# nucypher/nufhe

Measured on NVIDIA B200. Metric: bootstrapped gates/sec (NAND) at batch 4096 per GPU, higher is better.
Workload: dtype u64

## Files before the change

### nufhe_b200/csrc/br_fft.cuh

```cuda
#pragma once
#include "br_phases.cuh"
#include <math.h>
#include <string.h>

namespace nb {

constexpr int FFT_M = 512;
constexpr int FFT_STRIDE = FFT_M + FFT_M / 8;
constexpr int FFT_KEY_SPECTRA = 16;
constexpr int FFT_ROW_U64 = FFT_KEY_SPECTRA * FFT_M * 2;
constexpr double FFT_ROUND_MAGIC = 6755399441055744.0;
constexpr double FFT_DIGIT_BIAS = 4503599627370496.0 + 512.0;
constexpr double FFT_SQRT1_2 = 0.70710678118654752440;
NB_HDC double fft_cos16(int j)
{
    return j == 0 ? 1.0 : j == 1 ? 0.9807852804032304491262 : j == 2 ? 0.9238795325112867561282
         : j == 3 ? 0.8314696123025452370788 : j == 4 ? 0.7071067811865475244008 : j == 5 ? 0.5555702330196022247428
         : j == 6 ? 0.3826834323650897717285 : j == 7 ? 0.1950903220161282678483 : 0.0;
}

NB_HD int fft_pos(int i) { return i + (i >> 3); }

struct cplx { double re, im; };

// ... 72 lines not shown
#endif
}
NB_HD cplx ld_c_global(const cplx *p)
{
#if defined(__CUDA_ARCH__)
    const double2 t = __ldg(reinterpret_cast<const double2 *>(p));
    return {t.x, t.y};
#else
    return *p;
#endif
}

template <bool INV> NB_HD cplx c_rot8(cplx a)
{
    return INV ? cplx{d_mul(d_add(a.re, a.im), FFT_SQRT1_2), d_mul(d_sub(a.im, a.re), FFT_SQRT1_2)}
               : cplx{d_mul(d_sub(a.re, a.im), FFT_SQRT1_2), d_mul(d_add(a.re, a.im), FFT_SQRT1_2)};
}
template <bool INV> NB_HD cplx c_rot16(cplx a, int j0)
{
    if (j0 == 4) return c_rot8<INV>(a);
    return c_mul(a, cplx{fft_cos16(j0), INV ? -fft_cos16(8 - j0) : fft_cos16(8 - j0)});
}

template <bool INV> NB_HD void dft8(cplx *x)
{
    auto rot4 = [](cplx a) -> cplx { return INV ? cplx{a.im, -a.re} : cplx{-a.im, a.re}; };
    auto rot8 = [](cplx a) -> cplx { return c_rot8<INV>(a); };
    cplx a[4], b[4];
    for (int j = 0; j < 4; j++) { a[j] = c_add(x[j], x[j + 4]); b[j] = c_sub(x[j], x[j + 4]); }
    b[1] = rot8(b[1]); b[2] = rot4(b[2]); b[3] = rot4(rot8(b[3]));
    cplx a0 = c_add(a[0], a[2]), a1 = c_add(a[1], a[3]), a2 = c_sub(a[0], a[2]), a3 = rot4(c_sub(a[1], a[3]));
    cplx b0 = c_add(b[0], b[2]), b1 = c_add(b[1], b[3]), b2 = c_sub(b[0], b[2]), b3 = rot4(c_sub(b[1], b[3]));
    x[0] = c_add(a0, a1); x[4] = c_sub(a0, a1); x[2] = c_add(a2, a3); x[6] = c_sub(a2, a3);
    x[1] = c_add(b0, b1); x[5] = c_sub(b0, b1); x[3] = c_add(b2, b3); x[7] = c_sub(b2, b3);
}

struct FftTables {
    cplx tw[FFT_M];
    cplx tw2[64];
};

NB_HD void fft_load_tw1(int t, const FftTables &T, cplx *tw)
{
    for (int k0 = 0; k0 < 8; k0++) tw[k0] = ld_c(&T.tw[64 * k0 + t]);
}

NB_HD void fft_fwd1_store(int t, cplx *x, cplx *f, const cplx *tw)
{
    for (int j0 = 1; j0 < 8; j0++) x[j0] = c_rot16<false>(x[j0], j0);
    dft8<false>(x);
    for (int k0 = 0; k0 < 8; k0++) st_c(f + fft_pos(64 * k0 + t), c_mul(x[k0], tw[k0]));
}
NB_HD void fft_fwd2(int t, cplx *f, const FftTables &T)
{
    const int base = 64 * (t >> 3) + (t & 7), j2 = t & 7;
    cplx x[8];
    for (int j1 = 0; j1 < 8; j1++) x[j1] = ld_c(f + fft_pos(base + 8 * j1));
    dft8<false>(x);
    st_c(f + fft_pos(base), x[0]);
    for (int k1 = 1; k1 < 8; k1++) st_c(f + fft_pos(base + 8 * k1), c_mul(x[k1], T.tw2[k1 * 8 + j2]));
}
NB_HD void fft_fwd3(int t, cplx *f)
{
    cplx *g = f + fft_pos(8 * t);
    cplx x[8];
    for (int j2 = 0; j2 < 8; j2++) x[j2] = ld_c(g + j2);
    dft8<false>(x);
    for (int k2 = 0; k2 < 8; k2++) st_c(g + k2, x[k2]);
}
NB_HD void fft_inv3(int t, cplx *f, const FftTables &T)
{
    cplx *g = f + fft_pos(8 * t);
    const int k1 = t & 7;
    cplx x[8];
    for (int k2 = 0; k2 < 8; k2++) x[k2] = ld_c(g + k2);
    dft8<true>(x);
    st_c(g, x[0]);
    for (int j2 = 1; j2 < 8; j2++) st_c(g + j2, c_mul(x[j2], c_conj(T.tw2[j2 * 8 + k1])));
}
NB_HD void fft_inv2(int t, cplx *f)
{
    const int base = 64 * (t >> 3) + (t & 7);
    cplx x[8];
    for (int k1 = 0; k1 < 8; k1++) x[k1] = ld_c(f + fft_pos(base + 8 * k1));
    dft8<true>(x);
    for (int j1 = 0; j1 < 8; j1++) st_c(f + fft_pos(base + 8 * j1), x[j1]);
}
NB_HD void fft_inv1_load(int t, const cplx *f, const cplx *tw, cplx *x)
{
    for (int k0 = 0; k0 < 8; k0++) x[k0] = c_mul(ld_c(f + fft_pos(64 * k0 + t)), c_conj(tw[k0]));
    dft8<true>(x);
    for (int j0 = 1; j0 < 8; j0++) x[j0] = c_rot16<true>(x[j0], j0);
}


template <bool ROTATE>
NB_HD void fft_step_fwd1(int t, const i32 *acc, cplx *f2 , const FftTables &T, int a)
{
    const int ar = a & (NTT_N - 1);
    const bool flip = (a >> 10) & 1;
    u32 tv[16];
    for (int h = 0; h < 16; h++) {
        const int idx = 64 * (h & 7) + t + 512 * (h >> 3);
        const i32 c = ROTATE ? rotate_minus_one(acc, idx, ar, flip) : acc[idx];
        tv[h] = (u32)c + (0x80000000u + (1u << 21));
    }
    cplx tw[8];
    fft_load_tw1(t, T, tw);
#if defined(__CUDA_ARCH__)
#pragma unroll 1
#endif
    for (int j = 0; j < 2; j++) {
        const int sh = 22 - 10 * j;
        cplx x[8];
        for (int j0 = 0; j0 < 8; j0++) {
            const double lo = d_sub(d_from_u32_biased((tv[j0] >> sh) & 1023u), FFT_DIGIT_BIAS);
            const double hi = d_sub(d_from_u32_biased((tv[8 + j0] >> sh) & 1023u), FFT_DIGIT_BIAS);
            x[j0] = cplx{lo, hi};
        }
        fft_fwd1_store(t, x, f2 + j * FFT_STRIDE, tw);
    }
}

NB_HD void fft_step_mac(int i, cplx *w, int stride, int ct, const cplx *key)
{
    cplx k[16];
    for (int s = 0; s < 16; s++) k[s] = ld_c_global(key + s * FFT_M + i);
    const int pos = fft_pos(i);
    for (int c = 0; c < ct; c++) {
        cplx *f = w + c * stride + pos;
        cplx d[4];
        for (int q = 0; q < 4; q++) d[q] = ld_c(f + q * FFT_STRIDE);
        for (int o = 0; o < 4; o++) {
            const int mo = o >> 1, limb = o & 1;
            cplx acc = {0.0, 0.0};
            for (int q = 0; q < 4; q++) acc = c_mac(acc, d[q], k[(q * 2 + mo) * 2 + limb]);
            st_c(f + o * FFT_STRIDE, acc);
        }
    }
}

template <bool ACCUMULATE>
NB_HD void fft_step_inv1(int t, i32 *acc, const cplx *f2 , const FftTables &T,
                         double *err_max = nullptr)
{
    u32 r[16];
    for (int h = 0; h < 16; h++) r[h] = 0;
    cplx tw[8];
    fft_load_tw1(t, T, tw);
#if defined(__CUDA_ARCH__)
#pragma unroll 1
#endif
    for (int limb = 0; limb < 2; limb++) {
        cplx x[8];
        fft_inv1_load(t, f2 + limb * FFT_STRIDE, tw, x);
        const int sh = 16 * limb;
        for (int j0 = 0; j0 < 8; j0++) {
            const cplx y = x[j0];
            r[j0] += d_round_lo32(y.re) << sh;
            r[8 + j0] += d_round_lo32(y.im) << sh;
#if !defined(__CUDA_ARCH__)
            if (err_max) {
                const double e0 = fabs(y.re - nearbyint(y.re)), e1 = fabs(y.im - nearbyint(y.im));
                if (e0 > *err_max) *err_max = e0;
                if (e1 > *err_max) *err_max = e1;
            }
#endif
        }
    }
    for (int h = 0; h < 16; h++) {
        const int idx = 64 * (h & 7) + t + 512 * (h >> 3);
        const u32 v = r[h];
        acc[idx] = ACCUMULATE ? (i32)((u32)acc[idx] + v) : (i32)v;
    }
}

NB_HD void fft_key_phase1(int t, const i32 *k, int limb, cplx *f, const FftTables &T)
{
    cplx x[8];
    for (int j0 = 0; j0 < 8; j0++) {
        const int idx = 64 * j0 + t;
        double v[2];
        for (int h = 0; h < 2; h++) {
            const i32 c = k[idx + 512 * h];
            const i32 lo = (i32)(int16_t)(u32)c;
            const i32 hi = (i32)(((long long)c - lo) >> 16);
            v[h] = (double)(limb ? hi : lo);
        }
        x[j0] = cplx{v[0], v[1]};
    }
    cplx tw[8];
    fft_load_tw1(t, T, tw);
    fft_fwd1_store(t, x, f, tw);
}
NB_HD void fft_key_phase3_store(int t, cplx *f, cplx *out)
{
// ... 9 lines not shown
```

### nufhe_b200/csrc/capi.cu

```cuda
#include <cstdio>
#include <cstdlib>
#include <cstring>
#include <string>
#include <type_traits>
#include <nvtx3/nvToolsExt.h>
#include "../../include/nufhe_b200.h"
#include "kernels.cuh"
#include "fft_kernels.cuh"
#include "tables.h"

using namespace nb;

struct nb_ctx {
    int device;
    cudaStream_t stream;
    u64 *d_ph_fwd, *d_ph_inv;
    u64 *d_ones512;
    int sm_count;
    size_t wide_max;
    size_t wide2_max;
    size_t pair_max;
    int pair_async;
    int max_chunks;
    unsigned *d_sched;
    size_t sched_words;
    int32_t *d_state;
    size_t state_words;
    float *d_cv_blocks;
    size_t cv_words;
    int force_chunks;
    int stagger_cycles;
    int use_fft;
    FftTables *d_fft_tab;
    std::string err;
};

static int fail(nb_ctx *ctx, int code, const std::string &msg)
{
    if (ctx) ctx->err = msg;
    return code;
}

static int check(nb_ctx *ctx, cudaError_t e, const char *what)
{
    if (e == cudaSuccess) return NB_OK;
    return fail(ctx, NB_ECUDA, std::string(what) + ": " + cudaGetErrorString(e));
}

#define NB_TRY(expr)                         \
    do {                                     \
        int _rc = (expr);                    \
        if (_rc != NB_OK) return _rc;        \
    } while (0)

static int launch_check(nb_ctx *ctx, const char *what) { return check(ctx, cudaGetLastError(), what); }

// ... 13 lines not shown
};
struct NvtxRange {
    explicit NvtxRange(const char *name) { nvtxRangePushA(name); }
    ~NvtxRange() { nvtxRangePop(); }
};

#define NB_ON_DEVICE(ctx)                   \
    DeviceGuard _guard((ctx)->device);      \
    NB_TRY(check(ctx, _guard.err, "cudaSetDevice"))

extern "C" {

int nb_ctx_create(int device, void *stream, nb_ctx **out)
{
    if (!out) return NB_EINVAL;
    *out = nullptr;
    nb_ctx *ctx = new nb_ctx();
    ctx->device = device;
    ctx->stream = (cudaStream_t)stream;
    ctx->d_ph_fwd = ctx->d_ph_inv = ctx->d_ones512 = nullptr;
    ctx->d_sched = nullptr; ctx->d_state = nullptr; ctx->sched_words = ctx->state_words = 0;
    ctx->d_cv_blocks = nullptr; ctx->cv_words = 0;
    ctx->d_fft_tab = nullptr;
    *out = ctx;
    NB_ON_DEVICE(ctx);
    cudaDeviceProp prop;
    NB_TRY(check(ctx, cudaGetDeviceProperties(&prop, device), "cudaGetDeviceProperties"));
    ctx->sm_count = prop.multiProcessorCount;
    {
        const char *e = getenv("NUFHE_B200_MAX_CHUNKS");
        ctx->max_chunks = e ? atoi(e) : 50;
        if (ctx->max_chunks < 1) ctx->max_chunks = 1;
        e = getenv("NUFHE_B200_FORCE_CHUNKS");
        ctx->force_chunks = e ? atoi(e) : 0;
        e = getenv("NUFHE_B200_STAGGER");
        ctx->stagger_cycles = e ? atoi(e) : 12000;
        e = getenv("NUFHE_B200_FFT");
        ctx->use_fft = e ? atoi(e) : 1;
    }
    if (const char *e = getenv("NUFHE_B200_FORCE_RARE_PATH")) {
        if (atoi(e)) {
            const u32 zero = 0;
            NB_TRY(check(ctx, cudaMemcpyToSymbol(nb_c_canon_trigger, &zero, sizeof(zero)), "cudaMemcpyToSymbol"));
        }
    }
    if (prop.major < 10)
        return fail(ctx, NB_EUNSUPPORTED, "libnufhe_b200 is built for sm_100a only; device is sm_" +
                                              std::to_string(prop.major) + std::to_string(prop.minor));
    PhaseTables pt;
    NB_TRY(check(ctx, cudaMalloc(&ctx->d_ph_fwd, NTT_N * sizeof(u64)), "cudaMalloc"));
    NB_TRY(check(ctx, cudaMalloc(&ctx->d_ph_inv, NTT_N * sizeof(u64)), "cudaMalloc"));
    NB_TRY(check(ctx, cudaMemcpy(ctx->d_ph_fwd, pt.fwd.data(), NTT_N * sizeof(u64), cudaMemcpyHostToDevice), "memcpy"));
    NB_TRY(check(ctx, cudaMemcpy(ctx->d_ph_inv, pt.inv.data(), NTT_N * sizeof(u64), cudaMemcpyHostToDevice), "memcpy"));
    NB_TRY(check(ctx, cudaMalloc(&ctx->d_ones512, NTT_N * sizeof(u64)), "cudaMalloc"));
    NB_TRY(check(ctx, cudaMemcpy(ctx->d_ones512, pt.ones512.data(), NTT_N * sizeof(u64), cudaMemcpyHostToDevice), "memcpy"));
    {
        FftTables ft;
        make_fft_tables(ft);
        NB_TRY(check(ctx, cudaMalloc(&ctx->d_fft_tab, sizeof(FftTables)), "cudaMalloc"));
        NB_TRY(check(ctx, cudaMemcpy(ctx->d_fft_tab, &ft, sizeof(FftTables), cudaMemcpyHostToDevice), "memcpy"));
    }
    NB_TRY(check(ctx, cudaFuncSetAttribute(blind_rotate_fft_kernel<BrFft>, cudaFuncAttributeMaxDynamicSharedMemorySize,
                                           (int)br_fft_smem_bytes<BrFft>()), "cudaFuncSetAttribute(blind_rotate fft)"));
    NB_TRY(check(ctx, cudaFuncSetAttribute(blind_rotate_kernel<BrDefault>, cudaFuncAttributeMaxDynamicSharedMemorySize,
                                           (int)br_smem_bytes<BrDefault>()), "cudaFuncSetAttribute(blind_rotate)"));
    NB_TRY(check(ctx, cudaFuncSetAttribute(blind_rotate_kernel<BrWide>, cudaFuncAttributeMaxDynamicSharedMemorySize,
                                           (int)br_smem_bytes<BrWide>()), "cudaFuncSetAttribute(blind_rotate wide)"));
    NB_TRY(check(ctx, cudaFuncSetAttribute(blind_rotate_kernel<BrWide2>, cudaFuncAttributeMaxDynamicSharedMemorySize,
                                           (int)br_smem_bytes<BrWide2>()), "cudaFuncSetAttribute(blind_rotate wide2)"));
    NB_TRY(check(ctx, cudaFuncSetAttribute(blind_rotate_pair_kernel<true>, cudaFuncAttributeMaxDynamicSharedMemorySize,
                                           (int)BR_PAIR_SMEM_BYTES), "cudaFuncSetAttribute(blind_rotate pair)"));
    NB_TRY(check(ctx, cudaFuncSetAttribute(blind_rotate_pair_kernel<false>, cudaFuncAttributeMaxDynamicSharedMemorySize,
                                           (int)BR_PAIR_SMEM_BYTES), "cudaFuncSetAttribute(blind_rotate pair)"));
    NB_TRY(check(ctx, cudaFuncSetAttribute(keyswitch_kernel, cudaFuncAttributeMaxDynamicSharedMemorySize,
                                           (int)KS_SMEM_BYTES), "cudaFuncSetAttribute(keyswitch)"));
    {
        const char *e = getenv("NUFHE_B200_WIDE_MAX");
        ctx->wide_max = e ? (size_t)atoll(e) : (size_t)ctx->sm_count * BrWide::CTAS_PER_SM * 17 / 10;
        e = getenv("NUFHE_B200_WIDE2_MAX");
        ctx->wide2_max = e ? (size_t)atoll(e) : (size_t)ctx->sm_count * 3 / 2;
        e = getenv("NUFHE_B200_PAIR_ASYNC");
        ctx->pair_async = e ? atoi(e) : 1;
        e = getenv("NUFHE_B200_PAIR_MAX");
// ... 16 lines not shown
        }
        if (getenv("NUFHE_B200_VERBOSE"))
            fprintf(stderr, "nufhe_b200: device %d, %d SMs; fused-kernel shapes by batch: pair <= %zu, wide2 <= %zu, wide <= %zu\n",
                    ctx->device, ctx->sm_count, ctx->pair_max, ctx->wide2_max, ctx->wide_max);
    }
    NB_TRY(check(ctx, cudaFuncSetAttribute(ntt_forward_kernel<true>, cudaFuncAttributeMaxDynamicSharedMemorySize, (int)ntt_smem_bytes(NTT_RAW_I32_BYTES)), "attr"));
    NB_TRY(check(ctx, cudaFuncSetAttribute(ntt_forward_kernel<false>, cudaFuncAttributeMaxDynamicSharedMemorySize, (int)ntt_smem_bytes(NTT_RAW_U64_BYTES)), "attr"));
    NB_TRY(check(ctx, cudaFuncSetAttribute(ntt_inverse_kernel<true>, cudaFuncAttributeMaxDynamicSharedMemorySize, (int)ntt_smem_bytes(NTT_RAW_U64_BYTES)), "attr"));
    NB_TRY(check(ctx, cudaFuncSetAttribute(ntt_inverse_kernel<false>, cudaFuncAttributeMaxDynamicSharedMemorySize, (int)ntt_smem_bytes(NTT_RAW_U64_BYTES)), "attr"));
    return NB_OK;
}

void nb_ctx_destroy(nb_ctx *ctx)
{
    if (!ctx) return;
    DeviceGuard guard(ctx->device);
    if (ctx->d_ph_fwd) cudaFree(ctx->d_ph_fwd);
    if (ctx->d_ph_inv) cudaFree(ctx->d_ph_inv);
    if (ctx->d_ones512) cudaFree(ctx->d_ones512);
    if (ctx->d_sched) cudaFree(ctx->d_sched);
    if (ctx->d_state) cudaFree(ctx->d_state);
    if (ctx->d_cv_blocks) cudaFree(ctx->d_cv_blocks);
    if (ctx->d_fft_tab) cudaFree(ctx->d_fft_tab);
    delete ctx;
}

const char *nb_last_error(const nb_ctx *ctx) { return ctx ? ctx->err.c_str() : "null context"; }

int nb_ctx_set_stream(nb_ctx *ctx, void *stream)
{
    if (!ctx) return NB_EINVAL;
    ctx->stream = (cudaStream_t)stream;
    return NB_OK;
}

int nb_ctx_synchronize(nb_ctx *ctx)
{
    if (!ctx) return NB_EINVAL;
    NB_ON_DEVICE(ctx);
    return check(ctx, cudaStreamSynchronize(ctx->stream), "cudaStreamSynchronize");
}

const char *nb_build_info(void)
{
    static std::string info;
    if (info.empty()) {
// ... 148 lines not shown
template <class Cfg> static int launch_br_cfg(nb_ctx *ctx, BlindRotateArgs &p)
{
    const size_t slots = (size_t)ctx->sm_count * Cfg::CTAS_PER_SM;
    const size_t chains = (p.batch + Cfg::CT - 1) / Cfg::CT;
    int chunks = p.plain ? 1 : pick_chunks(chains, slots, p.n, ctx->max_chunks);
    if (!p.plain && ctx->force_chunks > 0 && chains > slots) chunks = ctx->force_chunks < p.n ? ctx->force_chunks : p.n;
    p.chains = (unsigned)chains;
    p.steps_per_chunk = p.plain ? 1 : (p.n + chunks - 1) / chunks;
    chunks = p.plain ? 1 : (p.n + p.steps_per_chunk - 1) / p.steps_per_chunk;
    p.chunks = (unsigned)chunks;
    p.sched = nullptr; p.state = nullptr;
    p.sm_count = ctx->sm_count; p.stagger_cycles = ctx->stagger_cycles;
    size_t grid = chains;
    if (chains > slots) {
        const size_t entries = chunks > 1 ? chains * (size_t)chunks : 0;
        NB_TRY(reserve_words(ctx, (void **)&ctx->d_sched, &ctx->sched_words, BR_SCHED_HEADER + entries, sizeof(unsigned)));
        if (chunks > 1)
            NB_TRY(reserve_words(ctx, (void **)&ctx->d_state, &ctx->state_words, chains * Cfg::CT * 2 * NTT_N, sizeof(int32_t)));
        NB_TRY(check(ctx, cudaMemsetAsync(ctx->d_sched, 0, (BR_SCHED_HEADER + entries) * sizeof(unsigned), ctx->stream), "cudaMemsetAsync"));
        p.sched = ctx->d_sched; p.state = ctx->d_state;
        grid = slots;
    }
    if constexpr (std::is_same_v<Cfg, BrFft>)
        blind_rotate_fft_kernel<Cfg><<<(int)grid, Cfg::THREADS, br_fft_smem_bytes<Cfg>(), ctx->stream>>>(p, ctx->d_fft_tab);
    else
        blind_rotate_kernel<Cfg><<<(int)grid, Cfg::THREADS, br_smem_bytes<Cfg>(), ctx->stream>>>(p, ctx->d_ph_fwd, ctx->d_ph_inv);
    return NB_OK;
}

static int launch_br(nb_ctx *ctx, BlindRotateArgs &p)
{
    if (!p.plain && p.n > 0 && p.batch <= ctx->pair_max) {
        p.sched = nullptr; p.state = nullptr; p.chains = (unsigned)p.batch; p.chunks = 1; p.steps_per_chunk = p.n;
        p.sm_count = ctx->sm_count; p.stagger_cycles = 0;
        if (ctx->pair_async) blind_rotate_pair_kernel<true><<<(unsigned)(2 * p.batch), PAIR_THREADS, BR_PAIR_SMEM_BYTES, ctx->stream>>>(p, ctx->d_ph_fwd, ctx->d_ph_inv);
        else blind_rotate_pair_kernel<false><<<(unsigned)(2 * p.batch), PAIR_THREADS, BR_PAIR_SMEM_BYTES, ctx->stream>>>(p, ctx->d_ph_fwd, ctx->d_ph_inv);
        return NB_OK;
    }
    if (p.batch <= ctx->wide2_max) return launch_br_cfg<BrWide2>(ctx, p);
    if (p.batch <= ctx->wide_max) return launch_br_cfg<BrWide>(ctx, p);
    if (ctx->use_fft && !p.plain && !p.bara && p.n > 0) return launch_br_cfg<BrFft>(ctx, p);
    return launch_br_cfg<BrDefault>(ctx, p);
}

extern "C" {

int nb_ctx_reserve(nb_ctx *ctx, size_t batch)
// ... 274 lines not shown
```

### nufhe_b200/csrc/fft_kernels.cuh

```cuda
#pragma once
#include "kernels.cuh"
#include "br_fft.cuh"

namespace nb {

template <int CT_> struct BrFftCfg {
    static constexpr int CT = CT_, THREADS = 128 * CT_;
    static constexpr int CTAS_PER_SM = CT_ <= 2 ? 2 : 1;
};
#ifndef NB_FFT_CT
#define NB_FFT_CT 2
#endif
using BrFft = BrFftCfg<NB_FFT_CT>;

template <class Cfg> constexpr size_t br_fft_smem_bytes()
{
    return (size_t)Cfg::CT * 4 * FFT_STRIDE * sizeof(cplx) + sizeof(FftTables) + (size_t)Cfg::CT * 2 * NTT_N * sizeof(i32) + 64;
}

enum { FFT_CLK_FWD1, FFT_CLK_FWD2, FFT_CLK_FWD3, FFT_CLK_MAC, FFT_CLK_INV3, FFT_CLK_INV2, FFT_CLK_INV1, FFT_CLK_SYNC,
       FFT_CLK_OTHER, FFT_CLK_STEPS, FFT_CLK_SLOTS };
#ifdef NB_FFT_PHASE_CLOCKS
constexpr int FFT_CLK_CTAS = 1024;
__device__ unsigned long long g_fft_phase_clocks[FFT_CLK_CTAS][FFT_CLK_SLOTS];
__shared__ unsigned long long s_fft_clk[FFT_CLK_SLOTS];
struct FftClocks {
    long long t = 0;
    NB_D void start() { t = clock64(); }
    NB_D void mark(int k) { const long long n = clock64(); if (threadIdx.x == 0) s_fft_clk[k] += n - t; t = n; }
    NB_D void flush(int tid)
    {
        if (tid == 0 && blockIdx.x < FFT_CLK_CTAS)
            for (int k = 0; k < FFT_CLK_SLOTS; k++) g_fft_phase_clocks[blockIdx.x][k] += s_fft_clk[k];
    }
};
#else
struct FftClocks {
    NB_D void start() {}
    NB_D void mark(int) {}
    NB_D void flush(int) {}
};
#endif

template <class Cfg>
NB_D void br_fft_step(cplx *w, const FftTables &T, i32 *acc, const int *rot, const cplx *__restrict__ key, int tid, FftClocks &clk)
{
    constexpr int TH = Cfg::THREADS;
    {
        const int pm = tid >> 6;
        fft_step_fwd1<true>(tid & 63, acc + pm * NTT_N, w + pm * 2 * FFT_STRIDE, T, rot[pm >> 1]);
    }
    clk.mark(FFT_CLK_FWD1);
    __syncthreads();
    clk.mark(FFT_CLK_SYNC);
#pragma unroll 1
    for (int it = 0; it < 2; it++) { const int task = it * TH + tid; fft_fwd2(task & 63, w + (task >> 6) * FFT_STRIDE, T); }
    clk.mark(FFT_CLK_FWD2);
    __syncthreads();
    clk.mark(FFT_CLK_SYNC);
#pragma unroll 1
    for (int it = 0; it < 2; it++) { const int task = it * TH + tid; fft_fwd3(task & 63, w + (task >> 6) * FFT_STRIDE); }
    clk.mark(FFT_CLK_FWD3);
    __syncthreads();
    clk.mark(FFT_CLK_SYNC);
#pragma unroll 1
    for (int i = tid; i < FFT_M; i += TH) fft_step_mac(i, w, 4 * FFT_STRIDE, Cfg::CT, key);
    clk.mark(FFT_CLK_MAC);
    __syncthreads();
    clk.mark(FFT_CLK_SYNC);
#pragma unroll 1
    for (int it = 0; it < 2; it++) { const int task = it * TH + tid; fft_inv3(task & 63, w + (task >> 6) * FFT_STRIDE, T); }
    clk.mark(FFT_CLK_INV3);
    __syncthreads();
    clk.mark(FFT_CLK_SYNC);
#pragma unroll 1
    for (int it = 0; it < 2; it++) { const int task = it * TH + tid; fft_inv2(task & 63, w + (task >> 6) * FFT_STRIDE); }
    clk.mark(FFT_CLK_INV2);
    __syncthreads();
    clk.mark(FFT_CLK_SYNC);
    {
        const int pp = tid >> 6;
        fft_step_inv1<true>(tid & 63, acc + pp * NTT_N, w + pp * 2 * FFT_STRIDE, T);
    }
    clk.mark(FFT_CLK_INV1);
}

template <class Cfg>
__global__ void __launch_bounds__(Cfg::THREADS, Cfg::CTAS_PER_SM) blind_rotate_fft_kernel(BlindRotateArgs p, const FftTables *__restrict__ tab_g)
{
    extern __shared__ __align__(16) unsigned char smem_raw[];
    cplx *w = reinterpret_cast<cplx *>(smem_raw);
    FftTables &T = *reinterpret_cast<FftTables *>(w + Cfg::CT * 4 * FFT_STRIDE);
    i32 *acc = reinterpret_cast<i32 *>(&T + 1);
    int *rot = reinterpret_cast<int *>(acc + Cfg::CT * 2 * NTT_N);
    __shared__ unsigned s_item, s_entry;
    const int tid = threadIdx.x;
    FftClocks clk;
#ifdef NB_FFT_PHASE_CLOCKS
    if (tid < FFT_CLK_SLOTS) s_fft_clk[tid] = 0;
#endif
    for (int i = tid; i < (int)(sizeof(FftTables) / 16); i += Cfg::THREADS)
        reinterpret_cast<double2 *>(&T)[i] = reinterpret_cast<const double2 *>(tab_g)[i];
    const cplx *key0 = reinterpret_cast<const cplx *>(p.bk + (size_t)p.n * BK_ROW_U64);
    constexpr int KEY_ROW_CPLX = FFT_KEY_SPECTRA * FFT_M;
    const unsigned total = p.chains * p.chunks;
    constexpr int ACC_WORDS = Cfg::CT * 2 * NTT_N;
    if (Cfg::CTAS_PER_SM > 1 && !p.sched && p.stagger_cycles > 0 && blockIdx.x >= (unsigned)p.sm_count) {
        if (tid == 0) {
            const long long t0 = clock64();
            while (clock64() - t0 < p.stagger_cycles) { }
        }
    }
    __syncthreads();

    for (unsigned item = blockIdx.x;; ) {
        if (p.sched) {
            __syncthreads();
            if (tid == 0) s_item = atomicAdd(p.sched, 1u);
            __syncthreads();
            item = s_item;
        }
        if (item >= total) break;
        unsigned chunk = 0, chain = item;
        if (p.sched && item >= p.chains) {
// ... 87 lines not shown
```

### nufhe_b200/csrc/host_emul.cpp

```cpp
#include <cstring>
#include <vector>
#include "tables.h"

using namespace nb;

extern "C" {

void emul_ntt_forward(const u64 *in, u64 *out, size_t batch)
{
    static PhaseTables T;
    std::vector<u64> w(NTT_SWEEP_POLYS * POLY_STRIDE);
    for (size_t b = 0; b < batch; b++) {
        for (int task = 0; task < 64; task++) {
            u64 x[16];
            for (int j1 = 0; j1 < 16; j1++) x[j1] = ff_canon(in[b * NTT_N + 64 * j1 + task]);
            phase_fwd1_generic(task, x, w.data(), T.fwd.data());
        }
        for (int row = 0; row < 16; row++) for (int g = 0; g < 4; g++) phase_fwd2(0, row, g, w.data());
        for (int row = 0; row < 16; row++) for (int u = 0; u < 4; u++) phase_fwd3(0, row, u, w.data());
        for (int k = 0; k < NTT_N; k++) out[b * NTT_N + k] = ff_canon(w[w_position_of_natural(k)]);
    }
}

void emul_ntt_inverse(const u64 *in, u64 *out, size_t batch)
// ... 197 lines not shown
{
    std::vector<u64> plain(NTT_N);
    std::vector<i32> k(NTT_N);
    std::vector<cplx> f(FFT_STRIDE);
    for (int m = 0; m < 8; m++) {
        for (int x = 0; x < NTT_N; x++) plain[x] = ff_mul(ff_canon(bk_ref_row[m * NTT_N + x]), FF_RINV);
        emul_ntt_inverse_i32(plain.data(), k.data(), 1);
        for (int limb = 0; limb < 2; limb++) {
            for (int t = 0; t < 64; t++) fft_key_phase1(t, k.data(), limb, f.data(), T);
            for (int t = 0; t < 64; t++) fft_fwd2(t, f.data(), T);
            for (int t = 0; t < 64; t++) fft_key_phase3_store(t, f.data(), out + (m * 2 + limb) * FFT_M);
        }
    }
}

static const FftTables &fft_tables()
{
    static FftTables T;
    static bool init = false;
    if (!init) { make_fft_tables(T); init = true; }
    return T;
}

extern "C" {

void emul_fft_tables(double *tw, double *cos16)
{
    memcpy(tw, &fft_tables(), sizeof(FftTables));
    for (int j = 0; j <= 8; j++) cos16[j] = fft_cos16(j);
}

void emul_fft_key_spectra(const u64 *bk_ref, u64 *out, size_t rows)
{
    for (size_t r = 0; r < rows; r++)
        fft_key_row(bk_ref + r * 8 * NTT_N, fft_tables(), reinterpret_cast<cplx *>(out + r * FFT_ROW_U64));
}

void emul_fft_step(i32 *acc, const u64 *bk_ref_row, const int *rot, int nct, double *err_max)
{
    const FftTables &T = fft_tables();
    std::vector<cplx> key(FFT_KEY_SPECTRA * FFT_M);
    fft_key_row(bk_ref_row, T, key.data());
    std::vector<cplx> w((size_t)nct * 4 * FFT_STRIDE);
    *err_max = 0;
    for (int c = 0; c < nct; c++)
        for (int mi = 0; mi < 2; mi++)
            for (int t = 0; t < 64; t++) {
                cplx *f2 = w.data() + (c * 4 + mi * 2) * FFT_STRIDE;
                if (rot) fft_step_fwd1<true>(t, acc + (c * 2 + mi) * NTT_N, f2, T, rot[c]);
                else fft_step_fwd1<false>(t, acc + (c * 2 + mi) * NTT_N, f2, T, 0);
            }
    for (int s = 0; s < nct * 4; s++) for (int t = 0; t < 64; t++) fft_fwd2(t, w.data() + s * FFT_STRIDE, T);
    for (int s = 0; s < nct * 4; s++) for (int t = 0; t < 64; t++) fft_fwd3(t, w.data() + s * FFT_STRIDE);
    for (int i = 0; i < FFT_M; i++) fft_step_mac(i, w.data(), 4 * FFT_STRIDE, nct, key.data());
    for (int s = 0; s < nct * 4; s++) for (int t = 0; t < 64; t++) fft_inv3(t, w.data() + s * FFT_STRIDE, T);
    for (int s = 0; s < nct * 4; s++) for (int t = 0; t < 64; t++) fft_inv2(t, w.data() + s * FFT_STRIDE);
    for (int c = 0; c < nct; c++)
        for (int mo = 0; mo < 2; mo++)
            for (int t = 0; t < 64; t++) {
                const cplx *f2 = w.data() + (c * 4 + mo * 2) * FFT_STRIDE;
                if (rot) fft_step_inv1<true>(t, acc + (c * 2 + mo) * NTT_N, f2, T, err_max);
                else fft_step_inv1<false>(t, acc + (c * 2 + mo) * NTT_N, f2, T, err_max);
            }
}

}
```

### nufhe_b200/csrc/tables.h

```cpp
#pragma once
#include <vector>
#include "ntt_lane.cuh"
#include "br_phases.cuh"
#include "br_fft.cuh"
#include <cmath>

namespace nb {

inline u64 h_mul(u64 a, u64 b) { return (u64)(((unsigned __int128)a * b) % FF_P); }
inline u64 h_pow(u64 a, u64 e) { u64 r = 1; while (e) { if (e & 1) r = h_mul(r, a); a = h_mul(a, a); e >>= 1; } return r; }
inline u64 h_inv(u64 a) { return h_pow(a, FF_P - 2); }

constexpr u64 ROOT_GEN = 0xa70dc47e4cbdf43fULL;

struct PhaseTables {
    std::vector<u64> fwd, inv;
    std::vector<u64> ones512;
    PhaseTables() : fwd(NTT_N), inv(NTT_N), ones512(NTT_N)
    {
        {
            const u64 psi0 = h_pow(ROOT_GEN, (1ULL << 32) / 2048);
            for (int k = 0; k < NTT_N; k++) {
                u64 r = h_pow(psi0, 2 * k + 1);
                u64 denom = (FF_P + 1 - r) % FF_P;
// ... 1 lines not shown
            }
        }
        const u64 psi = h_pow(ROOT_GEN, (1ULL << 32) / 2048);
        const u64 psi_inv = h_inv(psi), n_inv = h_inv(NTT_N);
        for (int row = 0; row < 16; row++)
            for (int j2 = 0; j2 < 64; j2++) {
                int e = w_twiddle_exponent(row, j2);
                fwd[row * 64 + j2] = h_pow(psi, e);
                inv[row * 64 + j2] = h_mul(h_pow(psi_inv, e), n_inv);
            }
    }
};

inline void make_fft_tables(FftTables &T)
{
    const long double pi = 3.141592653589793238462643383279502884L;
    auto w = [&](int m) { m &= FFT_M - 1; return cplx{(double)cosl(2 * pi * m / FFT_M), (double)sinl(2 * pi * m / FFT_M)}; };
    for (int m = 0; m < FFT_M; m++) {
        const int e = ((m & 63) * (1 + 4 * (m >> 6))) & (2 * NTT_N - 1);
        T.tw[m] = cplx{(double)cosl(pi * e / NTT_N), (double)sinl(pi * e / NTT_N)};
    }
    for (int m = 0; m < 64; m++) T.tw2[m] = w(8 * (m >> 3) * (m & 7));
}

}
```

Before: 99230.

## Restructure blind-rotate FFT as warp-local 16x32 decomposition with shuffles

Replaces the three-pass radix-8 FFT (fwd1/fwd2/fwd3 and inverse) with a two-pass 16x32 decomposition where each warp owns one polynomial. The second pass pairs lanes and exchanges half-results with shuffles, so the block-wide __syncthreads between FFT stages become __syncwarp. The inverse accumulates into acc with shared-memory atomicAdd instead of a read-modify-write, and it uses new twiddle tables, padding and a swizzled layout. Fewer block barriers and passes come at the cost of more registers per thread (16-point DFTs) and atomic traffic.

```diff
diff --git a/nufhe_b200/csrc/br_fft.cuh b/nufhe_b200/csrc/br_fft.cuh
--- a/nufhe_b200/csrc/br_fft.cuh
+++ b/nufhe_b200/csrc/br_fft.cuh
@@ -118,7 +118,7 @@
     return c_mul(a, cplx{fft_cos16(j0), INV ? -fft_cos16(8 - j0) : fft_cos16(8 - j0)});
 }
 
-template <bool INV> NB_HD void dft8(cplx *x)
+template <bool INV> NB_HD void dft8(cplx *x, double r = 1.0)
 {
     auto rot4 = [](cplx a) -> cplx { return INV ? cplx{a.im, -a.re} : cplx{-a.im, a.re}; };
     auto rot8 = [](cplx a) -> cplx { return c_rot8<INV>(a); };
@@ -127,8 +127,11 @@
     b[1] = rot8(b[1]); b[2] = rot4(b[2]); b[3] = rot4(rot8(b[3]));
     cplx a0 = c_add(a[0], a[2]), a1 = c_add(a[1], a[3]), a2 = c_sub(a[0], a[2]), a3 = rot4(c_sub(a[1], a[3]));
     cplx b0 = c_add(b[0], b[2]), b1 = c_add(b[1], b[3]), b2 = c_sub(b[0], b[2]), b3 = rot4(c_sub(b[1], b[3]));
-    x[0] = c_add(a0, a1); x[4] = c_sub(a0, a1); x[2] = c_add(a2, a3); x[6] = c_sub(a2, a3);
-    x[1] = c_add(b0, b1); x[5] = c_sub(b0, b1); x[3] = c_add(b2, b3); x[7] = c_sub(b2, b3);
+    auto bf = [&](int k, cplx u, cplx v) {
+        x[k] = {d_fma(r, v.re, u.re), d_fma(r, v.im, u.im)};
+        x[k + 4] = {d_fma(-r, v.re, u.re), d_fma(-r, v.im, u.im)};
+    };
+    bf(0, a0, a1); bf(2, a2, a3); bf(1, b0, b1); bf(3, b2, b3);
 }
 
 struct FftTables {
@@ -164,57 +167,92 @@
     dft8<false>(x);
     for (int k2 = 0; k2 < 8; k2++) st_c(g + k2, x[k2]);
 }
-NB_HD void fft_inv3(int t, cplx *f, const FftTables &T)
-{
-    cplx *g = f + fft_pos(8 * t);
-    const int k1 = t & 7;
-    cplx x[8];
-    for (int k2 = 0; k2 < 8; k2++) x[k2] = ld_c(g + k2);
-    dft8<true>(x);
-    st_c(g, x[0]);
-    for (int j2 = 1; j2 < 8; j2++) st_c(g + j2, c_mul(x[j2], c_conj(T.tw2[j2 * 8 + k1])));
-}
-NB_HD void fft_inv2(int t, cplx *f)
-{
-    const int base = 64 * (t >> 3) + (t & 7);
-    cplx x[8];
-    for (int k1 = 0; k1 < 8; k1++) x[k1] = ld_c(f + fft_pos(base + 8 * k1));
-    dft8<true>(x);
-    for (int j1 = 0; j1 < 8; j1++) st_c(f + fft_pos(base + 8 * j1), x[j1]);
-}
-NB_HD void fft_inv1_load(int t, const cplx *f, const cplx *tw, cplx *x)
-{
-    for (int k0 = 0; k0 < 8; k0++) x[k0] = c_mul(ld_c(f + fft_pos(64 * k0 + t)), c_conj(tw[k0]));
-    dft8<true>(x);
-    for (int j0 = 1; j0 < 8; j0++) x[j0] = c_rot16<true>(x[j0], j0);
-}
+
+constexpr int FFT_STEP_STRIDE = 548;
+NB_HD int fft_mid_pos(int k0, int j1) { return 34 * k0 + j1; }
+NB_HD int fft_step_pos(int i) { const int u = i >> 6; return i ^ (u & 1) ^ ((u & 2) << 1); }
+NB_HD int fft_stored_index(int k) { return 64 * (k & 7) + 8 * ((k >> 3) & 7) + (k >> 6); }
+
+NB_HDC double fft_cos32(int j)
+{
+    return j == 0 ? 1.0 : j == 1 ? 0.9951847266721969 : j == 2 ? 0.9807852804032304 : j == 3 ? 0.9569403357322088
+         : j == 4 ? 0.9238795325112867 : j == 5 ? 0.881921264348355 : j == 6 ? 0.8314696123025452
+         : j == 7 ? 0.773010453362737 : j == 8 ? 0.7071067811865476 : j == 9 ? 0.6343932841636455
+         : j == 10 ? 0.5555702330196022 : j == 11 ? 0.47139673682599764 : j == 12 ? 0.3826834323650898
+         : j == 13 ? 0.2902846772544624 : j == 14 ? 0.19509032201612828 : j == 15 ? 0.0980171403295606 : 0.0;
+}
+template <bool INV> NB_HD cplx c_rot32(cplx a, int j0)
+{
+    if (j0 == 8) return c_rot8<INV>(a);
+    return c_mul(a, cplx{fft_cos32(j0), INV ? -fft_cos32(16 - j0) : fft_cos32(16 - j0)});
+}
+template <bool INV> NB_HD cplx c_rot4(cplx a) { return INV ? cplx{a.im, -a.re} : cplx{-a.im, a.re}; }
+NB_HD cplx c_xsign(cplx a, unsigned long long m)
+{
+#if defined(__CUDA_ARCH__)
+    return {__longlong_as_double(__double_as_longlong(a.re) ^ (long long)m), __longlong_as_double(__double_as_longlong(a.im) ^ (long long)m)};
+#else
+    unsigned long long b[2];
+    memcpy(b, &a, 16);
+    b[0] ^= m; b[1] ^= m;
+    memcpy(&a, b, 16);
+    return a;
+#endif
+}
+
+template <bool INV> NB_HD void dft16(cplx *x, double r = 1.0, unsigned long long m = 0)
+{
+    cplx a[8], b[8];
+    for (int j = 0; j < 8; j++) { a[j] = c_add(x[j], x[j + 8]); b[j] = c_xsign(c_sub(x[j], x[j + 8]), m); }
+    b[1] = c_rot16<INV>(b[1], 2); b[2] = c_rot8<INV>(b[2]); b[3] = c_rot16<INV>(b[3], 6); b[4] = c_rot4<INV>(b[4]);
+    b[5] = c_rot4<INV>(c_rot16<INV>(b[5], 2)); b[6] = c_rot4<INV>(c_rot8<INV>(b[6]));
+    b[7] = c_rot4<INV>(c_rot16<INV>(b[7], 6));
+    dft8<INV>(a, r);
+    dft8<INV>(b, r);
+    for (int k = 0; k < 8; k++) { x[2 * k] = a[k]; x[2 * k + 1] = b[k]; }
+}
+
+struct FftStepTables {
+    cplx twa[FFT_M];
+};
 
 
 template <bool ROTATE>
-NB_HD void fft_step_fwd1(int t, const i32 *acc, cplx *f2 , const FftTables &T, int a)
+NB_HD void fft_step_fwd_a(int j1, int j, const i32 *acc, cplx *f , const FftStepTables &T, int a)
 {
     const int ar = a & (NTT_N - 1);
     const bool flip = (a >> 10) & 1;
-    u32 tv[16];
-    for (int h = 0; h < 16; h++) {
-        const int idx = 64 * (h & 7) + t + 512 * (h >> 3);
-        const i32 c = ROTATE ? rotate_minus_one(acc, idx, ar, flip) : acc[idx];
-        tv[h] = (u32)c + (0x80000000u + (1u << 21));
-    }
-    cplx tw[8];
-    fft_load_tw1(t, T, tw);
-#if defined(__CUDA_ARCH__)
-#pragma unroll 1
-#endif
-    for (int j = 0; j < 2; j++) {
-        const int sh = 22 - 10 * j;
-        cplx x[8];
-        for (int j0 = 0; j0 < 8; j0++) {
-            const double lo = d_sub(d_from_u32_biased((tv[j0] >> sh) & 1023u), FFT_DIGIT_BIAS);
-            const double hi = d_sub(d_from_u32_biased((tv[8 + j0] >> sh) & 1023u), FFT_DIGIT_BIAS);
-            x[j0] = cplx{lo, hi};
+    const int sh = 22 - 10 * j;
+    cplx x[16];
+    for (int j0 = 0; j0 < 16; j0++) {
+        double v[2];
+        for (int h = 0; h < 2; h++) {
+            const int idx = 32 * j0 + j1 + 512 * h;
+            const i32 c = ROTATE ? rotate_minus_one(acc, idx, ar, flip) : acc[idx];
+            v[h] = d_sub(d_from_u32_biased((((u32)c + (0x80000000u + (1u << 21))) >> sh) & 1023u), FFT_DIGIT_BIAS);
         }
-        fft_fwd1_store(t, x, f2 + j * FFT_STRIDE, tw);
+        x[j0] = cplx{v[0], v[1]};
+    }
+    for (int j0 = 1; j0 < 16; j0++) x[j0] = c_rot32<false>(x[j0], j0);
+    dft16<false>(x);
+    for (int k0 = 0; k0 < 16; k0++) st_c(f + fft_mid_pos(k0, j1), c_mul(x[k0], ld_c(&T.twa[32 * k0 + j1])));
+}
+
+NB_HD void fft_step_fwd_b_load(int k0, int p, const cplx *f, cplx *z)
+{
+    for (int m = 0; m < 16; m++) z[m] = ld_c(f + fft_mid_pos(k0, 2 * m + p));
+    dft16<false>(z, p ? -1.0 : 1.0);
+}
+NB_HD void fft_step_fwd_b_store(int k0, int p, cplx *f, const cplx *z, const cplx *recv)
+{
+    const double sg = p ? -1.0 : 1.0;
+    for (int i = 0; i < 8; i++) {
+        const cplx e = p ? recv[i] : z[i], o = p ? z[i] : recv[i];
+        const cplx t = i == 0 ? o : c_rot16<false>(o, i);
+        const double tr = p ? t.im : t.re, ti = p ? t.re : t.im;
+        const int k1 = i + 8 * p;
+        st_c(f + fft_step_pos(fft_stored_index(k0 + 16 * k1)), cplx{d_fma(sg, tr, e.re), d_add(e.im, ti)});
+        st_c(f + fft_step_pos(fft_stored_index(k0 + 16 * (k1 + 16))), cplx{d_fma(-sg, tr, e.re), d_sub(e.im, ti)});
     }
 }
 
@@ -222,52 +260,67 @@
 {
     cplx k[16];
     for (int s = 0; s < 16; s++) k[s] = ld_c_global(key + s * FFT_M + i);
-    const int pos = fft_pos(i);
+    const int pos = fft_step_pos(i);
     for (int c = 0; c < ct; c++) {
         cplx *f = w + c * stride + pos;
         cplx d[4];
-        for (int q = 0; q < 4; q++) d[q] = ld_c(f + q * FFT_STRIDE);
+        for (int q = 0; q < 4; q++) d[q] = ld_c(f + q * FFT_STEP_STRIDE);
         for (int o = 0; o < 4; o++) {
             const int mo = o >> 1, limb = o & 1;
             cplx acc = {0.0, 0.0};
             for (int q = 0; q < 4; q++) acc = c_mac(acc, d[q], k[(q * 2 + mo) * 2 + limb]);
-            st_c(f + o * FFT_STRIDE, acc);
+            st_c(f + o * FFT_STEP_STRIDE, acc);
         }
     }
 }
 
-template <bool ACCUMULATE>
-NB_HD void fft_step_inv1(int t, i32 *acc, const cplx *f2 , const FftTables &T,
-                         double *err_max = nullptr)
-{
-    u32 r[16];
-    for (int h = 0; h < 16; h++) r[h] = 0;
-    cplx tw[8];
-    fft_load_tw1(t, T, tw);
-#if defined(__CUDA_ARCH__)
-#pragma unroll 1
-#endif
-    for (int limb = 0; limb < 2; limb++) {
-        cplx x[8];
-        fft_inv1_load(t, f2 + limb * FFT_STRIDE, tw, x);
-        const int sh = 16 * limb;
-        for (int j0 = 0; j0 < 8; j0++) {
-            const cplx y = x[j0];
-            r[j0] += d_round_lo32(y.re) << sh;
-            r[8 + j0] += d_round_lo32(y.im) << sh;
+NB_HD void fft_step_inv_b_load(int k0, int p, const cplx *f, cplx *keep, cplx *send)
+{
+    for (int i = 0; i < 8; i++) {
+        const int r = i + 8 * p;
+        const cplx lo = ld_c(f + fft_step_pos(fft_stored_index(k0 + 16 * r)));
+        const cplx hi = ld_c(f + fft_step_pos(fft_stored_index(k0 + 16 * (r + 16))));
+        const cplx e = c_add(lo, hi), d = c_sub(lo, hi);
+        const cplx t = i == 0 ? d : c_rot16<true>(d, i);
+        const cplx o = p ? cplx{t.im, -t.re} : t;
+        keep[i] = p ? o : e;
+        send[i] = p ? e : o;
+    }
+}
+NB_HD void fft_step_inv_b_store(int k0, int p, cplx *f, const cplx *keep, const cplx *recv)
+{
+    cplx x[16];
+    for (int i = 0; i < 8; i++) { x[i] = keep[i]; x[8 + i] = recv[i]; }
+    dft16<true>(x, 1.0, (unsigned long long)p << 63);
+    for (int m = 0; m < 16; m++) st_c(f + fft_mid_pos(k0, 2 * m + p), x[m]);
+}
+
+NB_HD void acc_add(i32 *p, u32 v)
+{
+#if defined(__CUDA_ARCH__)
+    atomicAdd(reinterpret_cast<unsigned *>(p), v);
+#else
+    *p = (i32)((u32)*p + v);
+#endif
+}
+NB_HD void fft_step_inv_a(int j1, int limb, i32 *acc, const cplx *f , const FftStepTables &T,
+                          double *err_max = nullptr)
+{
+    cplx x[16];
+    for (int k0 = 0; k0 < 16; k0++) x[k0] = c_mul(ld_c(f + fft_mid_pos(k0, j1)), c_conj(ld_c(&T.twa[32 * k0 + j1])));
+    dft16<true>(x);
+    for (int j0 = 1; j0 < 16; j0++) x[j0] = c_rot32<true>(x[j0], j0);
+    const int sh = 16 * limb;
+    for (int j0 = 0; j0 < 16; j0++) {
+        acc_add(acc + 32 * j0 + j1, d_round_lo32(x[j0].re) << sh);
+        acc_add(acc + 32 * j0 + j1 + 512, d_round_lo32(x[j0].im) << sh);
 #if !defined(__CUDA_ARCH__)
-            if (err_max) {
-                const double e0 = fabs(y.re - nearbyint(y.re)), e1 = fabs(y.im - nearbyint(y.im));
-                if (e0 > *err_max) *err_max = e0;
-                if (e1 > *err_max) *err_max = e1;
-            }
-#endif
+        if (err_max) {
+            const double e0 = fabs(x[j0].re - nearbyint(x[j0].re)), e1 = fabs(x[j0].im - nearbyint(x[j0].im));
+            if (e0 > *err_max) *err_max = e0;
+            if (e1 > *err_max) *err_max = e1;
         }
-    }
-    for (int h = 0; h < 16; h++) {
-        const int idx = 64 * (h & 7) + t + 512 * (h >> 3);
-        const u32 v = r[h];
-        acc[idx] = ACCUMULATE ? (i32)((u32)acc[idx] + v) : (i32)v;
+#endif
     }
 }
 
diff --git a/nufhe_b200/csrc/capi.cu b/nufhe_b200/csrc/capi.cu
--- a/nufhe_b200/csrc/capi.cu
+++ b/nufhe_b200/csrc/capi.cu
@@ -32,6 +32,7 @@
     int stagger_cycles;
     int use_fft;
     FftTables *d_fft_tab;
+    FftStepTables *d_fft_step_tab;
     std::string err;
 };
 
@@ -91,6 +92,7 @@
     ctx->d_sched = nullptr; ctx->d_state = nullptr; ctx->sched_words = ctx->state_words = 0;
     ctx->d_cv_blocks = nullptr; ctx->cv_words = 0;
     ctx->d_fft_tab = nullptr;
+    ctx->d_fft_step_tab = nullptr;
     *out = ctx;
     NB_ON_DEVICE(ctx);
     cudaDeviceProp prop;
@@ -128,6 +130,10 @@
         make_fft_tables(ft);
         NB_TRY(check(ctx, cudaMalloc(&ctx->d_fft_tab, sizeof(FftTables)), "cudaMalloc"));
         NB_TRY(check(ctx, cudaMemcpy(ctx->d_fft_tab, &ft, sizeof(FftTables), cudaMemcpyHostToDevice), "memcpy"));
+        FftStepTables st;
+        make_fft_step_tables(st);
+        NB_TRY(check(ctx, cudaMalloc(&ctx->d_fft_step_tab, sizeof(FftStepTables)), "cudaMalloc"));
+        NB_TRY(check(ctx, cudaMemcpy(ctx->d_fft_step_tab, &st, sizeof(FftStepTables), cudaMemcpyHostToDevice), "memcpy"));
     }
     NB_TRY(check(ctx, cudaFuncSetAttribute(blind_rotate_fft_kernel<BrFft>, cudaFuncAttributeMaxDynamicSharedMemorySize,
                                            (int)br_fft_smem_bytes<BrFft>()), "cudaFuncSetAttribute(blind_rotate fft)"));
@@ -190,6 +196,7 @@
     if (ctx->d_state) cudaFree(ctx->d_state);
     if (ctx->d_cv_blocks) cudaFree(ctx->d_cv_blocks);
     if (ctx->d_fft_tab) cudaFree(ctx->d_fft_tab);
+    if (ctx->d_fft_step_tab) cudaFree(ctx->d_fft_step_tab);
     delete ctx;
 }
 
@@ -384,7 +391,7 @@
         grid = slots;
     }
     if constexpr (std::is_same_v<Cfg, BrFft>)
-        blind_rotate_fft_kernel<Cfg><<<(int)grid, Cfg::THREADS, br_fft_smem_bytes<Cfg>(), ctx->stream>>>(p, ctx->d_fft_tab);
+        blind_rotate_fft_kernel<Cfg><<<(int)grid, Cfg::THREADS, br_fft_smem_bytes<Cfg>(), ctx->stream>>>(p, ctx->d_fft_step_tab);
     else
         blind_rotate_kernel<Cfg><<<(int)grid, Cfg::THREADS, br_smem_bytes<Cfg>(), ctx->stream>>>(p, ctx->d_ph_fwd, ctx->d_ph_inv);
     return NB_OK;
diff --git a/nufhe_b200/csrc/fft_kernels.cuh b/nufhe_b200/csrc/fft_kernels.cuh
--- a/nufhe_b200/csrc/fft_kernels.cuh
+++ b/nufhe_b200/csrc/fft_kernels.cuh
@@ -15,11 +15,11 @@
 
 template <class Cfg> constexpr size_t br_fft_smem_bytes()
 {
-    return (size_t)Cfg::CT * 4 * FFT_STRIDE * sizeof(cplx) + sizeof(FftTables) + (size_t)Cfg::CT * 2 * NTT_N * sizeof(i32) + 64;
-}
-
-enum { FFT_CLK_FWD1, FFT_CLK_FWD2, FFT_CLK_FWD3, FFT_CLK_MAC, FFT_CLK_INV3, FFT_CLK_INV2, FFT_CLK_INV1, FFT_CLK_SYNC,
-       FFT_CLK_OTHER, FFT_CLK_STEPS, FFT_CLK_SLOTS };
+    return (size_t)Cfg::CT * 4 * FFT_STEP_STRIDE * sizeof(cplx) + sizeof(FftStepTables) + (size_t)Cfg::CT * 2 * NTT_N * sizeof(i32) + 64;
+}
+
+enum { FFT_CLK_FWD_A, FFT_CLK_FWD_B, FFT_CLK_MAC, FFT_CLK_INV_B, FFT_CLK_INV_A, FFT_CLK_SYNC, FFT_CLK_OTHER, FFT_CLK_STEPS,
+       FFT_CLK_SLOTS };
 #ifdef NB_FFT_PHASE_CLOCKS
 constexpr int FFT_CLK_CTAS = 1024;
 __device__ unsigned long long g_fft_phase_clocks[FFT_CLK_CTAS][FFT_CLK_SLOTS];
@@ -42,55 +42,59 @@
 };
 #endif
 
+NB_D cplx shfl_xor1(cplx v) { return {__shfl_xor_sync(0xffffffffu, v.re, 1), __shfl_xor_sync(0xffffffffu, v.im, 1)}; }
+
+NB_D void fft_step_fwd_b(int k0, int p, cplx *f)
+{
+    cplx z[16], recv[8];
+    fft_step_fwd_b_load(k0, p, f, z);
+    for (int i = 0; i < 8; i++) recv[i] = shfl_xor1(z[8 + i]);
+    __syncwarp();
+    fft_step_fwd_b_store(k0, p, f, z, recv);
+}
+NB_D void fft_step_inv_b(int k0, int p, cplx *f)
+{
+    cplx keep[8], send[8];
+    fft_step_inv_b_load(k0, p, f, keep, send);
+    for (int i = 0; i < 8; i++) send[i] = shfl_xor1(send[i]);
+    __syncwarp();
+    fft_step_inv_b_store(k0, p, f, keep, send);
+}
+
 template <class Cfg>
-NB_D void br_fft_step(cplx *w, const FftTables &T, i32 *acc, const int *rot, const cplx *__restrict__ key, int tid, FftClocks &clk)
+NB_D void br_fft_step(cplx *w, const FftStepTables &T, i32 *acc, const int *rot, const cplx *__restrict__ key, int tid, FftClocks &clk)
 {
     constexpr int TH = Cfg::THREADS;
-    {
-        const int pm = tid >> 6;
-        fft_step_fwd1<true>(tid & 63, acc + pm * NTT_N, w + pm * 2 * FFT_STRIDE, T, rot[pm >> 1]);
-    }
-    clk.mark(FFT_CLK_FWD1);
+    static_assert(TH == Cfg::CT * 4 * 32, "one warp per polynomial");
+    const int k0 = (tid >> 1) & 15, p = tid & 1;
+    cplx *wb = w + (tid >> 5) * FFT_STEP_STRIDE;
+    fft_step_fwd_a<true>(tid & 31, (tid >> 5) & 1, acc + (tid >> 6) * NTT_N, wb, T, rot[tid >> 7]);
+    clk.mark(FFT_CLK_FWD_A);
+    __syncwarp();
+    clk.mark(FFT_CLK_SYNC);
+    fft_step_fwd_b(k0, p, wb);
+    clk.mark(FFT_CLK_FWD_B);
     __syncthreads();
     clk.mark(FFT_CLK_SYNC);
 #pragma unroll 1
-    for (int it = 0; it < 2; it++) { const int task = it * TH + tid; fft_fwd2(task & 63, w + (task >> 6) * FFT_STRIDE, T); }
-    clk.mark(FFT_CLK_FWD2);
-    __syncthreads();
-    clk.mark(FFT_CLK_SYNC);
-#pragma unroll 1
-    for (int it = 0; it < 2; it++) { const int task = it * TH + tid; fft_fwd3(task & 63, w + (task >> 6) * FFT_STRIDE); }
-    clk.mark(FFT_CLK_FWD3);
-    __syncthreads();
-    clk.mark(FFT_CLK_SYNC);
-#pragma unroll 1
-    for (int i = tid; i < FFT_M; i += TH) fft_step_mac(i, w, 4 * FFT_STRIDE, Cfg::CT, key);
+    for (int i = tid; i < FFT_M; i += TH) fft_step_mac(i, w, 4 * FFT_STEP_STRIDE, Cfg::CT, key);
     clk.mark(FFT_CLK_MAC);
     __syncthreads();
     clk.mark(FFT_CLK_SYNC);
-#pragma unroll 1
-    for (int it = 0; it < 2; it++) { const int task = it * TH + tid; fft_inv3(task & 63, w + (task >> 6) * FFT_STRIDE, T); }
-    clk.mark(FFT_CLK_INV3);
-    __syncthreads();
-    clk.mark(FFT_CLK_SYNC);
-#pragma unroll 1
-    for (int it = 0; it < 2; it++) { const int task = it * TH + tid; fft_inv2(task & 63, w + (task >> 6) * FFT_STRIDE); }
-    clk.mark(FFT_CLK_INV2);
-    __syncthreads();
-    clk.mark(FFT_CLK_SYNC);
-    {
-        const int pp = tid >> 6;
-        fft_step_inv1<true>(tid & 63, acc + pp * NTT_N, w + pp * 2 * FFT_STRIDE, T);
-    }
-    clk.mark(FFT_CLK_INV1);
+    fft_step_inv_b(k0, p, wb);
+    clk.mark(FFT_CLK_INV_B);
+    __syncwarp();
+    clk.mark(FFT_CLK_SYNC);
+    fft_step_inv_a(tid & 31, (tid >> 5) & 1, acc + (tid >> 6) * NTT_N, wb, T);
+    clk.mark(FFT_CLK_INV_A);
 }
 
 template <class Cfg>
-__global__ void __launch_bounds__(Cfg::THREADS, Cfg::CTAS_PER_SM) blind_rotate_fft_kernel(BlindRotateArgs p, const FftTables *__restrict__ tab_g)
+__global__ void __launch_bounds__(Cfg::THREADS, Cfg::CTAS_PER_SM) blind_rotate_fft_kernel(BlindRotateArgs p, const FftStepTables *__restrict__ tab_g)
 {
     extern __shared__ __align__(16) unsigned char smem_raw[];
     cplx *w = reinterpret_cast<cplx *>(smem_raw);
-    FftTables &T = *reinterpret_cast<FftTables *>(w + Cfg::CT * 4 * FFT_STRIDE);
+    FftStepTables &T = *reinterpret_cast<FftStepTables *>(w + Cfg::CT * 4 * FFT_STEP_STRIDE);
     i32 *acc = reinterpret_cast<i32 *>(&T + 1);
     int *rot = reinterpret_cast<int *>(acc + Cfg::CT * 2 * NTT_N);
     __shared__ unsigned s_item, s_entry;
@@ -99,7 +103,7 @@
 #ifdef NB_FFT_PHASE_CLOCKS
     if (tid < FFT_CLK_SLOTS) s_fft_clk[tid] = 0;
 #endif
-    for (int i = tid; i < (int)(sizeof(FftTables) / 16); i += Cfg::THREADS)
+    for (int i = tid; i < (int)(sizeof(FftStepTables) / 16); i += Cfg::THREADS)
         reinterpret_cast<double2 *>(&T)[i] = reinterpret_cast<const double2 *>(tab_g)[i];
     const cplx *key0 = reinterpret_cast<const cplx *>(p.bk + (size_t)p.n * BK_ROW_U64);
     constexpr int KEY_ROW_CPLX = FFT_KEY_SPECTRA * FFT_M;
diff --git a/nufhe_b200/csrc/host_emul.cpp b/nufhe_b200/csrc/host_emul.cpp
--- a/nufhe_b200/csrc/host_emul.cpp
+++ b/nufhe_b200/csrc/host_emul.cpp
@@ -243,6 +243,28 @@
     return T;
 }
 
+static const FftStepTables &fft_step_tables()
+{
+    static FftStepTables T;
+    static bool init = false;
+    if (!init) { make_fft_step_tables(T); init = true; }
+    return T;
+}
+
+static void fft_step_fwd_b_warp(cplx *f)
+{
+    cplx z[32][16], recv[32][8];
+    for (int l = 0; l < 32; l++) fft_step_fwd_b_load(l >> 1, l & 1, f, z[l]);
+    for (int l = 0; l < 32; l++) for (int i = 0; i < 8; i++) recv[l][i] = z[l ^ 1][8 + i];
+    for (int l = 0; l < 32; l++) fft_step_fwd_b_store(l >> 1, l & 1, f, z[l], recv[l]);
+}
+static void fft_step_inv_b_warp(cplx *f)
+{
+    cplx keep[32][8], send[32][8];
+    for (int l = 0; l < 32; l++) fft_step_inv_b_load(l >> 1, l & 1, f, keep[l], send[l]);
+    for (int l = 0; l < 32; l++) fft_step_inv_b_store(l >> 1, l & 1, f, keep[l], send[l ^ 1]);
+}
+
 extern "C" {
 
 void emul_fft_tables(double *tw, double *cos16)
@@ -259,30 +281,45 @@
 
 void emul_fft_step(i32 *acc, const u64 *bk_ref_row, const int *rot, int nct, double *err_max)
 {
-    const FftTables &T = fft_tables();
+    const FftStepTables &T = fft_step_tables();
     std::vector<cplx> key(FFT_KEY_SPECTRA * FFT_M);
-    fft_key_row(bk_ref_row, T, key.data());
-    std::vector<cplx> w((size_t)nct * 4 * FFT_STRIDE);
+    fft_key_row(bk_ref_row, fft_tables(), key.data());
+    std::vector<cplx> w((size_t)nct * 4 * FFT_STEP_STRIDE);
     *err_max = 0;
-    for (int c = 0; c < nct; c++)
-        for (int mi = 0; mi < 2; mi++)
-            for (int t = 0; t < 64; t++) {
-                cplx *f2 = w.data() + (c * 4 + mi * 2) * FFT_STRIDE;
-                if (rot) fft_step_fwd1<true>(t, acc + (c * 2 + mi) * NTT_N, f2, T, rot[c]);
-                else fft_step_fwd1<false>(t, acc + (c * 2 + mi) * NTT_N, f2, T, 0);
-            }
-    for (int s = 0; s < nct * 4; s++) for (int t = 0; t < 64; t++) fft_fwd2(t, w.data() + s * FFT_STRIDE, T);
-    for (int s = 0; s < nct * 4; s++) for (int t = 0; t < 64; t++) fft_fwd3(t, w.data() + s * FFT_STRIDE);
-    for (int i = 0; i < FFT_M; i++) fft_step_mac(i, w.data(), 4 * FFT_STRIDE, nct, key.data());
-    for (int s = 0; s < nct * 4; s++) for (int t = 0; t < 64; t++) fft_inv3(t, w.data() + s * FFT_STRIDE, T);
-    for (int s = 0; s < nct * 4; s++) for (int t = 0; t < 64; t++) fft_inv2(t, w.data() + s * FFT_STRIDE);
-    for (int c = 0; c < nct; c++)
-        for (int mo = 0; mo < 2; mo++)
-            for (int t = 0; t < 64; t++) {
-                const cplx *f2 = w.data() + (c * 4 + mo * 2) * FFT_STRIDE;
-                if (rot) fft_step_inv1<true>(t, acc + (c * 2 + mo) * NTT_N, f2, T, err_max);
-                else fft_step_inv1<false>(t, acc + (c * 2 + mo) * NTT_N, f2, T, err_max);
-            }
-}
-
-}
+    for (int q = 0; q < nct * 4; q++)
+        for (int j1 = 0; j1 < 32; j1++) {
+            cplx *f = w.data() + q * FFT_STEP_STRIDE;
+            if (rot) fft_step_fwd_a<true>(j1, q & 1, acc + (q >> 1) * NTT_N, f, T, rot[q >> 2]);
+            else fft_step_fwd_a<false>(j1, q & 1, acc + (q >> 1) * NTT_N, f, T, 0);
+        }
+    for (int s = 0; s < nct * 4; s++) fft_step_fwd_b_warp(w.data() + s * FFT_STEP_STRIDE);
+    for (int i = 0; i < FFT_M; i++) fft_step_mac(i, w.data(), 4 * FFT_STEP_STRIDE, nct, key.data());
+    for (int s = 0; s < nct * 4; s++) fft_step_inv_b_warp(w.data() + s * FFT_STEP_STRIDE);
+    if (!rot) memset(acc, 0, sizeof(i32) * nct * 2 * NTT_N);
+    for (int q = 0; q < nct * 4; q++)
+        for (int j1 = 0; j1 < 32; j1++) fft_step_inv_a(j1, q & 1, acc + (q >> 1) * NTT_N, w.data() + q * FFT_STEP_STRIDE, T, err_max);
+}
+
+void emul_fft_step_tables(double *twa, double *cos32)
+{
+    memcpy(twa, &fft_step_tables(), sizeof(FftStepTables));
+    for (int j = 0; j <= 16; j++) cos32[j] = fft_cos32(j);
+}
+
+void emul_fft_step_forward(const i32 *poly, int digit, double *out)
+{
+    std::vector<cplx> w(FFT_STEP_STRIDE);
+    cplx *f = w.data();
+    for (int j1 = 0; j1 < 32; j1++) fft_step_fwd_a<false>(j1, digit, poly, f, fft_step_tables(), 0);
+    fft_step_fwd_b_warp(f);
+    for (int i = 0; i < FFT_M; i++) memcpy(out + 2 * i, f + fft_step_pos(i), sizeof(cplx));
+}
+
+int emul_fft_step_layout(int *mid, int *pos, int *stored)
+{
+    for (int k0 = 0; k0 < 16; k0++) for (int j1 = 0; j1 < 32; j1++) mid[32 * k0 + j1] = fft_mid_pos(k0, j1);
+    for (int i = 0; i < FFT_M; i++) { pos[i] = fft_step_pos(i); stored[i] = fft_stored_index(i); }
+    return FFT_STEP_STRIDE;
+}
+
+}
diff --git a/nufhe_b200/csrc/tables.h b/nufhe_b200/csrc/tables.h
--- a/nufhe_b200/csrc/tables.h
+++ b/nufhe_b200/csrc/tables.h
@@ -47,5 +47,13 @@
     }
     for (int m = 0; m < 64; m++) T.tw2[m] = w(8 * (m >> 3) * (m & 7));
 }
+inline void make_fft_step_tables(FftStepTables &T)
+{
+    const long double pi = 3.141592653589793238462643383279502884L;
+    for (int m = 0; m < FFT_M; m++) {
+        const int e = ((m & 31) * (1 + 4 * (m >> 5))) & (2 * NTT_N - 1);
+        T.twa[m] = cplx{(double)cosl(pi * e / NTT_N), (double)sinl(pi * e / NTT_N)};
+    }
+}
 
 }
```

After: 104,000, median of 6. 4.8% higher.
